# StanfordVL/RubiksNet

Hardware: AMD Instinct MI355X
Metric: RubiksShift3D fwd+bwd GB/s vs HBM roofline (higher is better)
Workload: dtype f32

## Files before the change

include/rubiks_hip.h:

```cpp
#ifndef RUBIKS_HIP_H_
#define RUBIKS_HIP_H_

#include <stddef.h>

#ifdef __cplusplus
extern "C" {
#endif

typedef void* rk_stream_t;

enum {
    RK_OK = 0,
    RK_ERR_NULL_POINTER = -1,
    RK_ERR_BAD_DIMS = -2,
    RK_ERR_BAD_STRIDE = -3,
    RK_ERR_WORKSPACE = -4,
    RK_ERR_LAUNCH = -5,
    RK_ERR_NO_DEVICE = -6,
    RK_ERR_UNSUPPORTED = -7
};

int rk_version(void);
const char* rk_error_string(int code);
int rk_out_len(int in, int stride, int pad);
// ... 238 lines not shown
                         int quantize, void* workspace, size_t workspace_bytes, rk_stream_t stream);
int rk_pw_tiles(int F, int P);
int rk_pw_gemm_tiles(const float* A, int F, int K, int M, int P, int a_is_mk);
int rk_pw2_gemm_cfg_f32(const float* A, const float* X, const float* R, float* Y, int F, int K, int M, int P, int a_is_mk,
                        const float* ka, const float* kb, int relu_in, int rb, int amode, int ct, rk_stream_t stream);
int rk_pw4_gemm_f32(const float* A, const float* X, const float* R, float* Y, int F, int K, int M, int P, int a_is_mk,
                    const float* ka, const float* kb, int relu_in, int epi, void* stats, const float* bx, const float* bpack,
                    void* bred, int tiles, rk_stream_t stream);
size_t rk_pw2_wgrad_workspace_bytes(int F, int K, int M, int P);
int rk_pw2_wgrad_cfg_f32(const float* dY, const float* X, float* dW, int F, int K, int M, int P, void* ws, size_t ws_bytes,
                         const float* ka, const float* kb, int relu_in, int inst, int stages, int splits, rk_stream_t stream);
int rk_pw_gemm_stats_f32(const float* A, const float* X, const float* R, float* Y, int F, int K, int M, int P,
                         int a_is_mk, const float* ka, const float* kb, int relu_in, void* stats, int tiles,
                         rk_stream_t stream);
int rk_stem_conv3x3s2_stats_f32(const float* W, const float* X, float* Y, int F, int Cin, int Cout, int Hin, int Win,
                                void* stats, int tiles, rk_stream_t stream);
int rk_pw_gemm_bnbwd_f32(const float* A, const float* dY, const float* R, float* dZ, int F, int K, int M, int P,
                         int a_is_mk, const float* x, const float* abmi , void* bred,
                         int tiles, rk_stream_t stream);
int rk_pw_wgrad_pro_f32(const float* dY, const float* X, float* dW, int F, int K, int M, int P, const float* ka,
                        const float* kb, int relu_in, void* ws, size_t ws_bytes, rk_stream_t stream);
int rk_pw_s2_wgrad_pro_f32(const float* dY, const float* X, float* dW, int F, int Cin, int Cout, int Hin, int Win,
                           const float* ka, const float* kb, int relu_in, void* ws, size_t ws_bytes, rk_stream_t stream);
int rk_bn_finish_tiles_f32(const void* stats, int tiles, long long count, const float* gamma, const float* beta,
                           float* running_mean, float* running_var, float* save_mean, float* save_invstd, float* a,
                           float* b, float* abmi , int C, float eps, float momentum,
                           long long* num_batches_tracked, rk_stream_t stream);
int rk_bn_tile_stats_f32(const float* x, void* stats, int F, int C, int P, rk_stream_t stream);
int rk_bn_apply_affine_bf16(const void* x, const float* a, const float* b, void* y, int F, int C, int P, int relu,
                            rk_stream_t stream);
int rk_bn_apply_affine_f32(const float* x, const float* a, const float* b, float* y, int F, int C, int P, int relu,
                           rk_stream_t stream);
int rk_bn_bwd_finish_tiles_f32(const void* bred, int tiles, long long count, float* k12, float* dgamma, float* dbeta,
                               int C, rk_stream_t stream);
int rk_bn_bwd_dx_pre_f32(const float* dz, const float* x, const float* gamma, const float* save_mean,
                         const float* save_invstd, const float* k12, const float* skip, float* dx, int F, int C, int P,
                         rk_stream_t stream);
int rk_bn_bwd_dx_pre_bf16(const void* dz, const void* x, const float* gamma, const float* save_mean,
                          const float* save_invstd, const float* k12, const void* skip, void* dx, int F, int C, int P,
                          rk_stream_t stream);
int rk_bn_stats_finish_f32(const float* x, const float* gamma, const float* beta, float* running_mean, float* running_var,
                           float* save_mean, float* save_invstd, float* ab, int F, int C, int P, float eps, float momentum,
                           long long* num_batches_tracked, void* ws, size_t ws_bytes, rk_stream_t stream);
int rk_bn_stats_finish_bf16(const void* x, const float* gamma, const float* beta, float* running_mean, float* running_var,
                            float* save_mean, float* save_invstd, float* ab, int F, int C, int P, float eps, float momentum,
                            long long* num_batches_tracked, void* ws, size_t ws_bytes, rk_stream_t stream);
// ... 34 lines not shown
```

rubiksnet_amd/_native.py:

```python
import ctypes
import os
import threading

_HERE = os.path.dirname(os.path.abspath(__file__))
LIB_PATH = os.environ.get("RK_HIP_LIB") or os.path.join(_HERE, "csrc", "librubiks_hip.so")

_lock = threading.Lock()
_lib = None

_i = ctypes.c_int
_p = ctypes.c_void_p
_sz = ctypes.c_size_t

_DIMS3 = [_i] * 5 + [_i] * 6
_DIMS2 = [_i] * 4 + [_i] * 4
SIGNATURES = {
    "rk_version": (_i, []),
    "rk_error_string": (ctypes.c_char_p, [_i]),
    "rk_out_len": (_i, [_i, _i, _i]),
    "rk_device_count": (_i, []),
    "rk_debug_peek_launch_tag": (ctypes.c_uint, []),
    "rk_debug_set_finalize_spins": (_i, [_i]),
    "rk3d_debug_finalize_only_f32": (_i, [_p, _sz, _i, _i, _p, _i, ctypes.c_float, _p]),
    "rk3d_forward_f32": (_i, [_p, _p, _p] + _DIMS3 + [_i, _p]),
# ... 58 lines not shown
    "rk_pw_wgrad_workspace_bytes": (_sz, [_i, _i, _i, _i]),
    "rk_pw2_gemm_cfg_f32": (_i, [_p, _p, _p, _p, _i, _i, _i, _i, _i, _p, _p, _i, _i, _i, _i, _p]),
    "rk_pw4_gemm_f32": (_i, [_p, _p, _p, _p, _i, _i, _i, _i, _i, _p, _p, _i, _i, _p, _p, _p, _p, _i, _p]),
    "rk_pw2_wgrad_workspace_bytes": (_sz, [_i, _i, _i, _i]),
    "rk_pw2_wgrad_cfg_f32": (_i, [_p, _p, _p, _i, _i, _i, _i, _p, _sz, _p, _p, _i, _i, _i, _i, _p]),
    "rk_pw_wgrad_f32": (_i, [_p, _p, _p, _i, _i, _i, _i, _p, _sz, _p]),
    "rk_pw_wgrad_bf16": (_i, [_p, _p, _p, _i, _i, _i, _i, _p, _sz, _p]),
    "rk_pw_gemm_odd_f32": (_i, [_p, _p, _p, _p, _i, _i, _i, _i, _i, _p]),
    "rk_pw_wgrad_odd_workspace_bytes": (_sz, [_i, _i, _i, _i]),
    "rk_pw_wgrad_odd_f32": (_i, [_p, _p, _p, _i, _i, _i, _i, _p, _sz, _p]),
    "rk_pw_s2_forward_odd_f32": (_i, [_p, _p, _p, _i, _i, _i, _i, _i, _p]),
    "rk_pw_s2_dgrad_odd_f32": (_i, [_p, _p, _p, _i, _i, _i, _i, _i, _p]),
    "rk_pw_s2_wgrad_odd_f32": (_i, [_p, _p, _p, _i, _i, _i, _i, _i, _p, _sz, _p]),
    "rk3d_forward_bn_f32": (_i, [_p, _p, _p, _p] + _DIMS3 + [_i, _p]),
    "rk3d_backward_bn_workspace_bytes": (_sz, _DIMS3),
    "rk3d_backward_bn_f32": (_i, [_p] * 9 + _DIMS3 + [_i, ctypes.c_float, _i, _p, _sz, _p]),
    "rk_pw_tiles": (_i, [_i, _i]),
    "rk_pw_gemm_tiles": (_i, [_p, _i, _i, _i, _i, _i]),
    "rk_pw_gemm_stats_f32": (_i, [_p, _p, _p, _p, _i, _i, _i, _i, _i, _p, _p, _i, _p, _i, _p]),
    "rk_stem_conv3x3s2_stats_f32": (_i, [_p, _p, _p, _i, _i, _i, _i, _i, _p, _i, _p]),
    "rk_pw_gemm_bnbwd_f32": (_i, [_p, _p, _p, _p, _i, _i, _i, _i, _i, _p, _p, _p, _i, _p]),
    "rk_pw_wgrad_pro_f32": (_i, [_p, _p, _p, _i, _i, _i, _i, _p, _p, _i, _p, _sz, _p]),
    "rk_pw_s2_wgrad_pro_f32": (_i, [_p, _p, _p, _i, _i, _i, _i, _i, _p, _p, _i, _p, _sz, _p]),
    "rk_bn_finish_tiles_f32": (_i, [_p, _i, ctypes.c_longlong, _p, _p, _p, _p, _p, _p, _p, _p, _p, _i, ctypes.c_float,
                                    ctypes.c_float, _p, _p]),
    "rk_bn_tile_stats_f32": (_i, [_p, _p, _i, _i, _i, _p]),
    "rk_bn_apply_affine_f32": (_i, [_p, _p, _p, _p, _i, _i, _i, _i, _p]),
    "rk_bn_apply_affine_bf16": (_i, [_p, _p, _p, _p, _i, _i, _i, _i, _p]),
    "rk_bn_bwd_finish_tiles_f32": (_i, [_p, _i, ctypes.c_longlong, _p, _p, _p, _i, _p]),
    "rk_bn_bwd_dx_pre_f32": (_i, [_p, _p, _p, _p, _p, _p, _p, _p, _i, _i, _i, _p]),
    "rk_bn_bwd_dx_pre_bf16": (_i, [_p, _p, _p, _p, _p, _p, _p, _p, _i, _i, _i, _p]),
    "rk_bn_stats_finish_f32": (_i, [_p, _p, _p, _p, _p, _p, _p, _p, _i, _i, _i, ctypes.c_float, ctypes.c_float, _p, _p, _sz, _p]),
    "rk_bn_stats_finish_bf16": (_i, [_p, _p, _p, _p, _p, _p, _p, _p, _i, _i, _i, ctypes.c_float, ctypes.c_float, _p, _p, _sz, _p]),
    "rk_bn_stats_finish_abmi_f32": (_i, [_p] * 9 + [_i, _i, _i, ctypes.c_float, ctypes.c_float, _p, _p, _sz, _p]),
    "rk_bn_stats_finish_abmi_bf16": (_i, [_p] * 9 + [_i, _i, _i, ctypes.c_float, ctypes.c_float, _p, _p, _sz, _p]),
}
SIGNATURES["rk_se_mlp_forward_f32"] = (_i, [_p, _p, _p, _p, _p, _i, _i, _i, _p])
SIGNATURES["rk_se_mlp_backward_f32"] = (_i, [_p] * 11 + [_i, _i, _i, _p])
SIGNATURES["rk_se_dgate_f32"] = (_i, [_p, _p, _p, _i, _i, _i, _p])
SIGNATURES["rk_se_scale_add_f32"] = (_i, [_p, _p, _p, ctypes.c_float, _p, _i, _i, _i, _p])
for _sfx in ("f32", "bf16"):
    SIGNATURES["rk_clip_u8_to_chw_" + _sfx] = (_i, [_p, _p, _p, _p, _i, _i, _i, _i, _p])
    SIGNATURES["rk_se_squeeze_" + _sfx] = (_i, [_p, _p, _i, _i, _i, _p])
    SIGNATURES["rk_se_scale_" + _sfx] = (_i, [_p, _p, _p, _i, _i, _i, _p])
    SIGNATURES["rk_se_scale_backward_" + _sfx] = (_i, [_p, _p, _p, _p, _p, _i, _i, _i, _p])
    SIGNATURES["rk_bn_relu_forward_" + _sfx] = (
# ... 53 lines not shown
```

rubiksnet_amd/csrc/rk_pw4.hip:

```cpp
#include <type_traits>
#include "rk_common.hpp"
#include "rk_dma.hpp"
#include "rk_pw4.hpp"

namespace rk {
namespace pw4 {

typedef float f32x4 __attribute__((ext_vector_type(4)));

struct Dims {
    int F, K, M, P;
    long long ntot;
    long long ntiles;
    int a_is_mk;
};

#ifndef RK_PW4_NT
#define RK_PW4_NT 2
#endif
#if RK_PW4_NT & 1
#define RK_PW4_LDNT " nt"
#else
#define RK_PW4_LDNT ""
#endif
__device__ __forceinline__ void dma16v(const void* p, unsigned lds_dst_uniform) {
    unsigned keep;
    asm volatile(
        "s_mov_b32 %0, m0\n\t"
        "s_mov_b32 m0, %2\n\t"
        "s_waitcnt lgkmcnt(0)\n\t"
        "global_load_lds_dwordx4 %1, off" RK_PW4_LDNT "\n\t"
        "s_mov_b32 m0, %0"
        : "=&s"(keep)
        : "v"(p), "s"(lds_dst_uniform)
        : "memory");
}
__device__ __forceinline__ float row16_sum_to_lane15(float v) {
// ... 25 lines not shown
    int n = 0;
    for (int u = a; u <= b; ++u) {
        int uu = u;
        if (u < 0) {
            if (first) continue;
            uu = u + NRT;
        }
        if (ne0) n += uu == NRT - 1 ? 4 * (RB - 1) * ns : 0;
        else if (uu >= NST && uu < NST + NE && (uu - NST) / 4 < RB - 1) n += ns;
    }
    return n;
}
constexpr int best_div(int n, int maxrec) {
    for (int dd = maxrec; dd >= 2; --dd)
        if (n % dd == 0) return dd;
    return 1;
}
constexpr int pad_of(int n, int maxrec) {
    for (int p = 0; p < 8; ++p)
        if (best_div(n + p, maxrec) >= 8) return p;
    return 0;
}
constexpr int maxrec_of(bool ALDS) { return ALDS ? 17 : 19; }

template <int RB, int NST, bool PRO, int EPI, bool RES, bool ALDS>
__global__ __launch_bounds__(64 * waves_of(ALDS), ALDS ? 1 : 2) void k_pw4_gemm(const float* __restrict__ A, const float* __restrict__ X,
                                                             const float* __restrict__ R, float* __restrict__ Y, Dims d,
                                                             pw2::GFuse fz, pw2::GTrain tr) {
    static_assert(!(EPI == 2 && (RES || PRO)), "no such instance");
    constexpr int NE = (EPI == 2 || RES) ? 4 * RB : 0;
    constexpr int NPAD = pad_of(NST + NE, maxrec_of(ALDS));
    constexpr int NRT = NST + NE + NPAD;
    constexpr int NREC = best_div(NRT, maxrec_of(ALDS));
    constexpr int LOOK = NREC - 1;
    constexpr int NS = EPI == 0 ? 1 : 2;
    static_assert(LOOK >= 2 && LOOK <= NRT, "ring");
    constexpr int kWaves = waves_of(ALDS);
    extern __shared__ __attribute__((aligned(16))) float lds_f[];
    const int wave = __builtin_amdgcn_readfirstlane((int)(threadIdx.x >> 6)), lane = threadIdx.x & 63;
    const int j = lane & 15, kq = lane >> 4;
    float* ring = lds_f + wave * (NREC * 256);
    float2* Ks = reinterpret_cast<float2*>(lds_f + kWaves * NREC * 256);
    float4* Bp = reinterpret_cast<float4*>(lds_f + kWaves * NREC * 256 + 8 * NST);
    float* At = lds_f + kWaves * NREC * 256 + 8 * NST + 64 * RB;
    const int K = d.K, M = d.M, P = d.P;
    if constexpr (ALDS) {
        for (int e = threadIdx.x; e < RB * NST * 64; e += 64 * kWaves) {
            const int l = e & 63, fs = e >> 6, st = fs % NST, rb = fs / NST;
            const int m = 16 * rb + (l & 15), k = 4 * st + (l >> 4);
            const bool ok = m < M && k < K;
            const size_t at = d.a_is_mk ? (size_t)m * K + k : (size_t)k * M + m;
            const float v = A[ok ? at : 0];
            At[e] = ok ? v : 0.f;
        }
    }
    if constexpr (PRO) {
        for (int e = threadIdx.x; e < 4 * NST; e += 64 * kWaves)
            Ks[e] = e < K ? make_float2(fz.ka[e], fz.kb[e]) : make_float2(0.f, 0.f);
    }
    if constexpr (EPI == 2) {
        for (int e = threadIdx.x; e < 16 * RB; e += 64 * kWaves) Bp[e] = tr.bpack[e < M ? e : M - 1];
    }
    const bool outaff = EPI == 0 && fz.ma != nullptr;
    if (outaff) {
        for (int e = threadIdx.x; e < 16 * RB; e += 64 * kWaves) {
            const int m = e < M ? e : M - 1;
            Bp[e] = make_float4(fz.ma[m], fz.mb[m], 0.f, 0.f);
        }
    }
    if (PRO || EPI == 2 || ALDS || outaff) __syncthreads();

    const int gw = blockIdx.x * kWaves + wave, nwv = gridDim.x * kWaves;
    if (gw >= d.ntiles) return;
    const int ntw = (int)((d.ntiles - gw + nwv - 1) / nwv);

    const float* E = EPI == 2 ? tr.bx : R;
    const unsigned cstep = 64u * (unsigned)nwv, df = cstep / (unsigned)P, dp = cstep - df * (unsigned)P;
    unsigned pf_, pp_;
    {
        unsigned c = (unsigned)gw * 64u + 4u * (unsigned)j;
        c = c < (unsigned)d.ntot ? c : 0u;
        pf_ = c / (unsigned)P; pp_ = c - pf_ * (unsigned)P;
    }
    int ptile = 0;
    const unsigned ring_b = dma::lds_byte_addr(ring);
    const size_t kqP = (size_t)kq * P;
    int xfix;
    {
        const int k = 4 * (NST - 1) + kq;
        xfix = ((k < K ? k : K - 1) - k) * P;
    }
    const float* xp = nullptr;
    const float* ep = nullptr;
    size_t yo_next = 0;
    auto enter_tile = [&]() {
        const unsigned f = (pf_ * (unsigned)P + pp_) < (unsigned)d.ntot ? pf_ : 0u, p = f == pf_ ? pp_ : 0u;
        xp = X + ((size_t)f * K) * P + p + kqP;
        yo_next = ((size_t)f * M) * P + p;
        if constexpr (NE > 0) ep = E + yo_next + 4 * kqP;
// ... 37 lines not shown
    static_for<LOOK>([&](auto I) { issue(I); });
    size_t yo_c = yo_next, yo_next_c = yo_next;

    float a[ALDS ? 1 : RB][ALDS ? 1 : NST];
    if constexpr (!ALDS) {
#pragma unroll
        for (int rb = 0; rb < RB; ++rb)
#pragma unroll
            for (int st = 0; st < NST; ++st) {
                const int m = 16 * rb + j, k = 4 * st + kq;
                const bool ok = m < M && k < K;
                const size_t at = d.a_is_mk ? (size_t)m * K + k : (size_t)k * M + m;
                const float v = A[ok ? at : 0];
                a[rb][st] = ok ? v : 0.f;
            }
    }
    float acur[RB];
    auto read_a = [&](auto STc, float (&dst)[RB]) {
        constexpr int st = decltype(STc)::value;
#pragma unroll
        for (int rb = 0; rb < RB; ++rb) dst[rb] = At[(rb * NST + st) * 64 + lane];
    };
    if constexpr (ALDS) read_a(std::integral_constant<int, 0>{}, acur);

    asm volatile("s_waitcnt vmcnt(%0)" ::"n"(LOOK - 1) : "memory");
    f32x4 vcur = read_rec(std::integral_constant<int, 0>{});

    int t = 0;
    auto tile_body = [&](auto FIRSTc) {
        constexpr bool FIRST = decltype(FIRSTc)::value;
        const long long tg = (long long)gw + (long long)t * nwv;
        const bool valid = tg * 64 + 4 * j < d.ntot;
        const long long nleft = d.ntot - tg * 64;
        const float ntile = (float)(nleft < 64 ? nleft : 64);
        float* yp = Y + yo_c + 4 * kqP;
        size_t rec = (size_t)(4 * kq) * tr.J + (size_t)tg;
        auto finish_row = [&](auto RBc, auto Rc, const f32x4& ev) {
            constexpr int rb = decltype(RBc)::value, r = decltype(Rc)::value;
            const int m = 16 * rb + 4 * kq + r;
            const bool live = rb < RB - 1 || m < M;
            const bool on = valid && live;
            float4 o = make_float4(acc[rb][0][r], acc[rb][1][r], acc[rb][2][r], acc[rb][3][r]);
            if constexpr (EPI == 0) {
                if (outaff) {
                    const float4 pk = Bp[16 * rb + 4 * kq + r];
                    o.x = fmaf(pk.x, o.x, pk.y); o.y = fmaf(pk.x, o.y, pk.y); o.z = fmaf(pk.x, o.z, pk.y); o.w = fmaf(pk.x, o.w, pk.y);
// ... 18 lines not shown
                    const float4 pk = Bp[16 * rb + 4 * kq + r];
                    if (on) {
                        const float pa = pk.x, pb = pk.y, mu = pk.z, iv = pk.w;
                        o.x = fmaf(pa, ev[0], pb) <= 0.f ? 0.f : o.x;  s1 += o.x;  s2 = fmaf(o.x, (ev[0] - mu) * iv, s2);
                        o.y = fmaf(pa, ev[1], pb) <= 0.f ? 0.f : o.y;  s1 += o.y;  s2 = fmaf(o.y, (ev[1] - mu) * iv, s2);
                        o.z = fmaf(pa, ev[2], pb) <= 0.f ? 0.f : o.z;  s1 += o.z;  s2 = fmaf(o.z, (ev[2] - mu) * iv, s2);
                        o.w = fmaf(pa, ev[3], pb) <= 0.f ? 0.f : o.w;  s1 += o.w;  s2 = fmaf(o.w, (ev[3] - mu) * iv, s2);
                    }
                }
                if (on) store_y(yp, o);
                s1 = row16_sum_to_lane15(s1);
                s2 = row16_sum_to_lane15(s2);
                if (j == 15 && live) {
                    if constexpr (EPI == 1) tr.stats[rec] = make_float4(piv, s1, s2, ntile);
                    else tr.bred[rec] = make_float2(s1, s2);
                }
                rec += (r == 3 ? 13 : 1) * (size_t)tr.J;
            }
            yp += (r == 3 ? 13 : 1) * (size_t)P;
        };

        static_for<NRT>([&](auto S) {
            constexpr int s = decltype(S)::value;
            issue(std::integral_constant<int, (s + LOOK) % NRT>{});
            if constexpr ((s + LOOK) % NRT == 0) yo_next_c = yo_next;
            constexpr int W = (LOOK - 1) + certain_stores(s + 1 - LOOK, s - 1, FIRST, NRT, NST, NE, RB, NS);
            static_assert(W <= 63, "vmcnt is 6 bits");
            asm volatile("s_waitcnt vmcnt(%0)" ::"n"(W) : "memory");
            const f32x4 vnext = read_rec(std::integral_constant<int, (s + 1) % NRT>{});
            const f32x4 v = vcur;
            float anext[RB];
            if constexpr (ALDS && ((s + 1) % NRT) < NST) read_a(std::integral_constant<int, (s + 1) % NRT>{}, anext);
            if constexpr (s < NST) {
                float b[4] = {v[0], v[1], v[2], v[3]};
                if constexpr (PRO) {
                    const float2 kk = Ks[4 * s + kq];
#pragma unroll
                    for (int q = 0; q < 4; ++q) {
                        const float tq = fmaf(kk.x, b[q], kk.y);
                        b[q] = fz.relu_in ? fmaxf(tq, 0.f) : tq;
                    }
                }
#pragma unroll
                for (int rb = 0; rb < RB; ++rb)
#pragma unroll
                    for (int q = 0; q < 4; ++q)
// ... 2 lines not shown
                constexpr int e = s - NST;
                finish_row(std::integral_constant<int, e / 4>{}, std::integral_constant<int, e % 4>{}, v);
            }
            vcur = vnext;
            if constexpr (ALDS && ((s + 1) % NRT) < NST) {
#pragma unroll
                for (int rb = 0; rb < RB; ++rb) acur[rb] = anext[rb];
            }
        });
        if constexpr (NE == 0) {
            static_for<4 * RB>([&](auto Ec) {
                constexpr int e = decltype(Ec)::value;
                finish_row(std::integral_constant<int, e / 4>{}, std::integral_constant<int, e % 4>{}, f32x4{0.f, 0.f, 0.f, 0.f});
            });
        }
#pragma unroll
        for (int rb = 0; rb < RB; ++rb)
#pragma unroll
            for (int q = 0; q < 4; ++q) acc[rb][q] = f32x4{0.f, 0.f, 0.f, 0.f};
        yo_c = yo_next_c;
    };
    tile_body(std::true_type{});
    for (t = 1; t < ntw; ++t) tile_body(std::false_type{});
}

struct Inst { int rb, nst; };
inline bool pick(Inst& in, int K, int M) {
    const int nrb = (M + 15) / 16, nst = (K + 3) / 4;
    if (nrb == 4 && nst >= 12 && nst <= 14) { in = Inst{4, 14}; return true; }
    if (nrb == 5 && nst >= 16 && nst <= 18) { in = Inst{5, 18}; return true; }
    return false;
}
inline int mode() {
    static const int m = [] { const char* e = getenv("RK_PW4"); return e ? atoi(e) : 1; }();
    return m;
}
inline int num_cus() { return device_cus(); }
constexpr long long kMinTiles = 4096;

template <int RB, int NST, bool PRO, int EPI, bool RES>
int launch(const float* A, const float* X, const float* R, float* Y, const Dims& d, const pw2::GFuse& fz, const pw2::GTrain& tr,
           hipStream_t stream) {
    constexpr bool ALDS = RB == 5 && EPI != 0;
    constexpr int NE = (EPI == 2 || RES) ? 4 * RB : 0;
    constexpr int NREC = best_div(NST + NE + pad_of(NST + NE, maxrec_of(ALDS)), maxrec_of(ALDS));
    constexpr int kWaves = waves_of(ALDS);
    if ((long long)d.F * d.K * d.P < 256) return RK_ERR_UNSUPPORTED;
    constexpr int wgs_per_cu = ALDS ? 1 : 2;
    const size_t lds = (size_t)kWaves * NREC * 1024 + 8 * NST * sizeof(float) + 16 * RB * sizeof(float4) +
                       (ALDS ? (size_t)RB * NST * 256 : 0);
    if (lds > 160 * 1024) return RK_ERR_UNSUPPORTED;
    static DynLdsRaised raised;
    if (const int rc = raise_dynamic_lds(reinterpret_cast<const void*>(&k_pw4_gemm<RB, NST, PRO, EPI, RES, ALDS>), lds, raised))
        return rc;
    long long wgs = (long long)num_cus() * wgs_per_cu;
    const long long need = (d.ntiles + kWaves - 1) / kWaves;
    wgs = wgs < need ? wgs : need;
    hipLaunchKernelGGL((k_pw4_gemm<RB, NST, PRO, EPI, RES, ALDS>), dim3((unsigned)wgs), dim3(64 * kWaves), lds, stream, A, X, R, Y, d,
                       fz, tr);
    return launch_status();
}
template <int RB, int NST>
int launch_flags(int pro, int epi, int res, const float* A, const float* X, const float* R, float* Y, const Dims& d,
                 const pw2::GFuse& fz, const pw2::GTrain& tr, hipStream_t stream) {
    if (epi == 2) {
        if (pro || res) return RK_ERR_UNSUPPORTED;
        return launch<RB, NST, false, 2, false>(A, X, R, Y, d, fz, tr, stream);
    }
#define RK_P4(E) do { \
        if (pro) return res ? launch<RB, NST, true, E, true>(A, X, R, Y, d, fz, tr, stream) \
                            : launch<RB, NST, true, E, false>(A, X, R, Y, d, fz, tr, stream); \
        return res ? launch<RB, NST, false, E, true>(A, X, R, Y, d, fz, tr, stream) \
                   : launch<RB, NST, false, E, false>(A, X, R, Y, d, fz, tr, stream); } while (0)
    if (epi == 1) RK_P4(1);
    RK_P4(0);
#undef RK_P4
}

long long tiles(int F, int K, int M, int P, int epi, int res, bool force) {
    if (F <= 0 || K <= 0 || M <= 0 || P <= 0 || P % 4 != 0 || (long long)F * P >= (1ll << 31)) return 0;
    if (mode() == 0) return 0;
    Inst in;
    if (!pick(in, K, M)) return 0;
    const long long nt = ((long long)F * P + 63) / 64;
    if (!force && mode() != 2) {
        if (nt < kMinTiles) return 0;
        if (in.rb == 5 && epi == 1 && res) return 0;
    }
    return nt;
}

int gemm(const float* A, const float* X, const float* R, float* Y, int F, int K, int M, int P, int a_is_mk, const pw2::GFuse* fuse,
         const pw2::GTrain* train, int epi, hipStream_t stream, bool force) {
    if (!A || !X || !Y) return RK_ERR_NULL_POINTER;
    if (F <= 0 || K <= 0 || M <= 0 || P <= 0 || P % 4 != 0) return RK_ERR_BAD_DIMS;
    if (((uintptr_t)X & 15) || ((uintptr_t)Y & 15) || (R && ((uintptr_t)R & 15))) return RK_ERR_BAD_DIMS;
    Inst in;
    if (!pick(in, K, M)) return RK_ERR_UNSUPPORTED;
    if (tiles(F, K, M, P, epi, R != nullptr, force) <= 0) return RK_ERR_UNSUPPORTED;
    pw2::GFuse fz = fuse ? *fuse : pw2::GFuse{nullptr, nullptr, nullptr, nullptr, 0, 0};
    pw2::GTrain tr = train ? *train : pw2::GTrain{nullptr, nullptr, nullptr, nullptr, 0};
    if (fz.ma && (epi != 0 || !fz.mb)) return RK_ERR_UNSUPPORTED;
    const int pro = fz.ka != nullptr, res = R != nullptr;
    Dims d;
    d.F = F; d.K = K; d.M = M; d.P = P; d.ntot = (long long)F * P; d.ntiles = (d.ntot + 63) / 64; d.a_is_mk = a_is_mk;
    if (epi == 1 && !tr.stats) return RK_ERR_NULL_POINTER;
    if (epi == 2 && !(tr.bred && tr.bx && tr.bpack)) return RK_ERR_NULL_POINTER;
    if (epi == 2 && ((uintptr_t)tr.bx & 15)) return RK_ERR_BAD_DIMS;
    if (epi && (long long)tr.J != d.ntiles) return RK_ERR_BAD_DIMS;
    if (in.rb == 4) return launch_flags<4, 14>(pro, epi, res, A, X, R, Y, d, fz, tr, stream);
    return launch_flags<5, 18>(pro, epi, res, A, X, R, Y, d, fz, tr, stream);
}

}
}

extern "C" {
using namespace rk;
int rk_pw4_gemm_f32(const float* A, const float* X, const float* R, float* Y, int F, int K, int M, int P, int a_is_mk,
                    const float* ka, const float* kb, int relu_in, int epi, void* stats, const float* bx, const float* bpack,
                    void* bred, int tiles, rk_stream_t stream) {
    const pw2::GFuse fz{ka, kb, nullptr, nullptr, relu_in, 0};
    const pw2::GTrain tr{(float4*)stats, (float2*)bred, bx, (const float4*)bpack, tiles};
    return pw4::gemm(A, X, R, Y, F, K, M, P, a_is_mk, &fz, &tr, epi, (hipStream_t)stream, true);
}
}
```

rubiksnet_amd/train_block.py:

```python
import logging

import torch

from . import _native, config, rubiksnet_cuda
from .fused_bn import _count_batch

__all__ = ["fused_train_block", "take_stats", "bn_relu_from_stats", "stats_fallbacks"]

_LOG = logging.getLogger("rubiksnet_amd")
_FALLBACKS = [0]


def stats_fallbacks():
    return _FALLBACKS[0]


def _note_fallback(shape):
    _FALLBACKS[0] += 1
    if _FALLBACKS[0] == 1:
        _LOG.warning("rubiksnet_amd: a fused training block received x %s without its producer's BatchNorm tile statistics "
                     "and runs a statistics pass of its own (logged once; train_block.stats_fallbacks() counts them)",
                     tuple(shape))

_CMAX = 320
# ... 210 lines not shown
        s3, pd = [1, plan.stride, plan.stride], [0, 0, 0]
        if dout is None:
            return (None,) * 13
        dout = dout.contiguous()
        need = ctx.needs_input_grad
        with torch.cuda.device(dev):
            st = _stream(dev)
            cur = torch.cuda.current_stream(dev)
            side = _side_stream(dev)
            keep = []

            def wgrad_ws(K, M, Pn):
                nbytes = int(L.rk_pw_wgrad_workspace_bytes(Fr, K, M, Pn))
                buf = torch.empty(max(nbytes, 1), dtype=torch.uint8, device=dev)
                keep.append(buf)
                return buf, nbytes

            def wg_stream():
                if side is None:
                    return st
                side.wait_stream(cur)
                return side.cuda_stream

            try:
                ds = torch.empty_like(s)
                _native.check(L.rk_pw_gemm_f32(w3.data_ptr(), dout.data_ptr(), None, ds.data_ptr(), Fr, Cout, Cmid, Po, 0, st),
                              "rk_pw_gemm_f32")
                dw3 = None
                if need[8]:
                    dw3 = torch.empty_like(w3)
                    ws, nb = wgrad_ws(Cmid, Cout, Po)
                    _native.check(L.rk_pw_wgrad_f32(dout.data_ptr(), (s_in if ctx.has_se else s).data_ptr(), dw3.data_ptr(), Fr,
                                                    Cmid, Cout, Po, ws.data_ptr(), nb, wg_stream()), "rk_pw_wgrad_f32")
                if ctx.has_se:
                    dgate = torch.empty_like(se_g)
                    _native.check(L.rk_se_dgate_f32(ds.data_ptr(), s.data_ptr(), dgate.data_ptr(), Fr, Cmid, Po, st),
                                  "rk_se_dgate_f32")
                    Cr = wse1.shape[0]
                    dpre2 = torch.empty_like(se_g)
                    dpre1 = torch.empty_like(se_h)
                    dq = torch.empty_like(se_g)
                    dwse1, dwse2 = torch.empty_like(wse1), torch.empty_like(wse2)
                    rc = L.rk_se_mlp_backward_f32(dgate.data_ptr(), se_g.data_ptr(), se_h.data_ptr(), se_q.data_ptr(), wse1.data_ptr(),
                                                  wse2.data_ptr(), dpre2.data_ptr(), dpre1.data_ptr(), dq.data_ptr(), dwse1.data_ptr(),
                                                  dwse2.data_ptr(), Fr, Cmid, Cr, st)
                    if rc == rubiksnet_cuda.UNSUPPORTED:
                        dpre2 = dgate * se_g * (1.0 - se_g)
                        dwse2 = dpre2.t() @ se_h
                        dpre1 = (dpre2 @ wse2) * (se_h > 0).to(dpre2.dtype)
                        dwse1 = dpre1.t() @ se_q
                        dq = (dpre1 @ wse1).contiguous()
                    else:
# ... 39 lines not shown
                if not need[7]:
                    dshift = None
                res, dwsc = None, None
                if not plan.identity:
                    res = torch.empty_like(x)
                    if plan.stride == 2:
                        _native.check(L.rk_pw_s2_dgrad_f32(wsc.data_ptr(), dout.data_ptr(), res.data_ptr(), Fr, Cin, Cout, H, W,
                                                           st), "rk_pw_s2_dgrad_f32")
                    else:
                        _native.check(L.rk_pw_gemm_f32(wsc.data_ptr(), dout.data_ptr(), None, res.data_ptr(), Fr, Cout, Cin, P,
                                                       0, st), "rk_pw_gemm_f32")
                    if need[9]:
                        dwsc = torch.empty_like(wsc)
                        ws, nb = wgrad_ws(Cin, Cout, Po)
                        if plan.stride == 2:
                            _native.check(L.rk_pw_s2_wgrad_pro_f32(dout.data_ptr(), x.data_ptr(), dwsc.data_ptr(), Fr, Cin, Cout,
                                                                   H, W, bn1[2].data_ptr(), bn1[3].data_ptr(), 1, ws.data_ptr(),
                                                                   nb, wg_stream()), "rk_pw_s2_wgrad_pro_f32")
                        else:
                            _native.check(L.rk_pw_wgrad_pro_f32(dout.data_ptr(), x.data_ptr(), dwsc.data_ptr(), Fr, Cin, Cout, P,
                                                                bn1[2].data_ptr(), bn1[3].data_ptr(), 1, ws.data_ptr(), nb,
                                                                wg_stream()), "rk_pw_wgrad_pro_f32")
                dw2 = None
                if need[4]:
                    dw2 = torch.empty_like(w2)
                    ws, nb = wgrad_ws(Cin, Cmid, P)
                    _native.check(L.rk_pw_wgrad_pro_f32(dz.data_ptr(), x.data_ptr(), dw2.data_ptr(), Fr, Cin, Cmid, P,
                                                        bn1[2].data_ptr(), bn1[3].data_ptr(), 1, ws.data_ptr(), nb, wg_stream()),
                                  "rk_pw_wgrad_pro_f32")
                J = int(L.rk_pw_gemm_tiles(w2.data_ptr(), Fr, Cmid, Cin, P, 0))
                bred = torch.empty(Cin, J, 2, dtype=torch.float32, device=dev)
                dzm = res if res is not None else torch.empty_like(x)
                _native.check(L.rk_pw_gemm_bnbwd_f32(w2.data_ptr(), dz.data_ptr(), _ptr(res), dzm.data_ptr(), Fr, Cmid, Cin, P,
                                                     0, x.data_ptr(), bn1[4].data_ptr(), bred.data_ptr(), J, st),
                              "rk_pw_gemm_bnbwd_f32")
                k12 = torch.empty(2, Cin, dtype=torch.float32, device=dev)
                dg1 = torch.empty(Cin, dtype=torch.float32, device=dev)
                db1 = torch.empty(Cin, dtype=torch.float32, device=dev)
                _native.check(L.rk_bn_bwd_finish_tiles_f32(bred.data_ptr(), J, Fr * P, k12.data_ptr(), dg1.data_ptr(),
                                                           db1.data_ptr(), Cin, st), "rk_bn_bwd_finish_tiles_f32")
                dx = None
                if need[0]:
                    dx = torch.empty_like(x)
                    skip = dout if plan.identity else None
                    _native.check(L.rk_bn_bwd_dx_pre_f32(dzm.data_ptr(), x.data_ptr(), g1.data_ptr(), bn1[0].data_ptr(),
                                                         bn1[1].data_ptr(), k12.data_ptr(), _ptr(skip), dx.data_ptr(), Fr, Cin,
                                                         P, st), "rk_bn_bwd_dx_pre_f32")
            finally:
                if side is not None:
                    cur.wait_stream(side)
                del keep
        return (dx, None, dg1, db1, dw2, dg2, db2, dshift, dw3, dwsc if not plan.identity else None, dwse1, dwse2, None)


def fused_train_block(block, x):
    sw = config.switches()
    if not (sw.fused_train and sw.fused_bn and sw.pointwise != "0"):
        return None
# ... 91 lines not shown
```

Before: 5821.

## Fuse pointwise dgrad GEMM with weight-gradient accumulation in backward pass

Adds a WG variant of the pw4 GEMM kernel. While streaming dY tiles to compute dX, it also reads the matching activation (E) tiles from the ring buffer and accumulates the weight gradient with MFMA into per-wave partials, which a reduce kernel then sums. The training block uses this fused path for the w3 and w2 (BN-backward with prologue affine) backward GEMMs by default, falling back when unsupported. This removes the separate wgrad kernel's re-read of dY and X from HBM. In exchange, occupancy drops to one workgroup per CU, register pressure rises, the partial workspace is extra traffic, and the wgrad no longer runs overlapped on a side stream.

After: 5816 (median of 6 runs). Within noise of the previous version (-0.1%).

```diff
diff --git a/include/rubiks_hip.h b/include/rubiks_hip.h
--- a/include/rubiks_hip.h
+++ b/include/rubiks_hip.h
@@ -284,6 +284,17 @@
                         const float* kb, int relu_in, void* ws, size_t ws_bytes, rk_stream_t stream);
 int rk_pw_s2_wgrad_pro_f32(const float* dY, const float* X, float* dW, int F, int Cin, int Cout, int Hin, int Win,
                            const float* ka, const float* kb, int relu_in, void* ws, size_t ws_bytes, rk_stream_t stream);
+size_t rk_pw_gemm_wgrad_workspace_bytes(int F, int K, int M, int P);
+int rk_pw_gemm_wgrad_f32(const float* A, const float* dY, float* dZ, int F, int K, int M, int P, int a_is_mk, const float* X,
+                         float* dW, void* ws, size_t ws_bytes, rk_stream_t stream);
+size_t rk_pw_gemm_bnbwd_wgrad_pro_workspace_bytes(int F, int K, int M, int P);
+int rk_pw_gemm_bnbwd_wgrad_pro_f32(const float* A, const float* dY, float* dZ, int F, int K, int M, int P, int a_is_mk,
+                                   const float* x, const float* abmi, void* bred, int tiles, const float* ka, const float* kb,
+                                   int relu_in, float* dW, void* ws, size_t ws_bytes, rk_stream_t stream);
+size_t rk_pw4_gemm_wgrad_workspace_bytes(int F, int K, int M, int P);
+int rk_pw4_gemm_wgrad_f32(const float* A, const float* dY, float* dZ, int F, int K, int M, int P, int a_is_mk, const float* bx,
+                          const float* abmi, void* bred, int tiles, const float* E, const float* ka, const float* kb, int relu_in,
+                          float* dW, void* ws, size_t ws_bytes, rk_stream_t stream);
 int rk_bn_finish_tiles_f32(const void* stats, int tiles, long long count, const float* gamma, const float* beta,
                            float* running_mean, float* running_var, float* save_mean, float* save_invstd, float* a,
                            float* b, float* abmi , int C, float eps, float momentum,
diff --git a/rubiksnet_amd/_native.py b/rubiksnet_amd/_native.py
--- a/rubiksnet_amd/_native.py
+++ b/rubiksnet_amd/_native.py
@@ -104,6 +104,12 @@
     "rk_pw_gemm_bnbwd_f32": (_i, [_p, _p, _p, _p, _i, _i, _i, _i, _i, _p, _p, _p, _i, _p]),
     "rk_pw_wgrad_pro_f32": (_i, [_p, _p, _p, _i, _i, _i, _i, _p, _p, _i, _p, _sz, _p]),
     "rk_pw_s2_wgrad_pro_f32": (_i, [_p, _p, _p, _i, _i, _i, _i, _i, _p, _p, _i, _p, _sz, _p]),
+    "rk_pw_gemm_wgrad_workspace_bytes": (_sz, [_i, _i, _i, _i]),
+    "rk_pw_gemm_wgrad_f32": (_i, [_p, _p, _p, _i, _i, _i, _i, _i, _p, _p, _p, _sz, _p]),
+    "rk_pw_gemm_bnbwd_wgrad_pro_workspace_bytes": (_sz, [_i, _i, _i, _i]),
+    "rk_pw_gemm_bnbwd_wgrad_pro_f32": (_i, [_p, _p, _p, _i, _i, _i, _i, _i, _p, _p, _p, _i, _p, _p, _i, _p, _p, _sz, _p]),
+    "rk_pw4_gemm_wgrad_workspace_bytes": (_sz, [_i, _i, _i, _i]),
+    "rk_pw4_gemm_wgrad_f32": (_i, [_p, _p, _p, _i, _i, _i, _i, _i, _p, _p, _p, _i, _p, _p, _p, _i, _p, _p, _sz, _p]),
     "rk_bn_finish_tiles_f32": (_i, [_p, _i, ctypes.c_longlong, _p, _p, _p, _p, _p, _p, _p, _p, _p, _i, ctypes.c_float,
                                     ctypes.c_float, _p, _p]),
     "rk_bn_tile_stats_f32": (_i, [_p, _p, _i, _i, _i, _p]),
diff --git a/rubiksnet_amd/csrc/rk_pw4.hip b/rubiksnet_amd/csrc/rk_pw4.hip
--- a/rubiksnet_amd/csrc/rk_pw4.hip
+++ b/rubiksnet_amd/csrc/rk_pw4.hip
@@ -2,6 +2,7 @@
 #include "rk_common.hpp"
 #include "rk_dma.hpp"
 #include "rk_pw4.hpp"
+#include "rk_reduce.hpp"
 
 namespace rk {
 namespace pw4 {
@@ -13,6 +14,12 @@
     long long ntot;
     long long ntiles;
     int a_is_mk;
+};
+struct WgArgs {
+    const float* E;
+    const float* ka; const float* kb;
+    int relu_in;
+    float* part;
 };
 
 #ifndef RK_PW4_NT
@@ -84,17 +91,21 @@
     return 0;
 }
 constexpr int maxrec_of(bool ALDS) { return ALDS ? 17 : 19; }
-
-template <int RB, int NST, bool PRO, int EPI, bool RES, bool ALDS>
-__global__ __launch_bounds__(64 * waves_of(ALDS), ALDS ? 1 : 2) void k_pw4_gemm(const float* __restrict__ A, const float* __restrict__ X,
+constexpr int maxrec_of(bool ALDS, int WG) { return WG ? 32 : maxrec_of(ALDS); }
+
+template <int RB, int NST, bool PRO, int EPI, bool RES, bool ALDS, int WG = 0>
+__global__ __launch_bounds__(64 * waves_of(ALDS), (ALDS || WG) ? 1 : 2) void k_pw4_gemm(const float* __restrict__ A, const float* __restrict__ X,
                                                              const float* __restrict__ R, float* __restrict__ Y, Dims d,
-                                                             pw2::GFuse fz, pw2::GTrain tr) {
+                                                             pw2::GFuse fz, pw2::GTrain tr, WgArgs wg) {
     static_assert(!(EPI == 2 && (RES || PRO)), "no such instance");
-    constexpr int NE = (EPI == 2 || RES) ? 4 * RB : 0;
-    constexpr int NPAD = pad_of(NST + NE, maxrec_of(ALDS));
+    static_assert(!(WG && (PRO || RES || ALDS || EPI == 1)), "no such instance");
+    constexpr int NE = (EPI == 2 || RES || WG) ? 4 * RB : 0;
+    constexpr int NPAD = pad_of(NST + NE, maxrec_of(ALDS, WG));
     constexpr int NRT = NST + NE + NPAD;
-    constexpr int NREC = best_div(NRT, maxrec_of(ALDS));
-    constexpr int LOOK = NREC - 1;
+    constexpr int NREC = best_div(NRT, maxrec_of(ALDS, WG));
+    constexpr int LOOK = WG ? NREC - 3 : NREC - 1;
+    constexpr int KB = (NST + 3) / 4;
+    static_assert(!WG || NPAD == 0, "WG: no padding records");
     constexpr int NS = EPI == 0 ? 1 : 2;
     static_assert(LOOK >= 2 && LOOK <= NRT, "ring");
     constexpr int kWaves = waves_of(ALDS);
@@ -105,6 +116,7 @@
     float2* Ks = reinterpret_cast<float2*>(lds_f + kWaves * NREC * 256);
     float4* Bp = reinterpret_cast<float4*>(lds_f + kWaves * NREC * 256 + 8 * NST);
     float* At = lds_f + kWaves * NREC * 256 + 8 * NST + 64 * RB;
+    float2* Kw = reinterpret_cast<float2*>(lds_f + kWaves * NREC * 256 + 8 * NST + 64 * RB);
     const int K = d.K, M = d.M, P = d.P;
     if constexpr (ALDS) {
         for (int e = threadIdx.x; e < RB * NST * 64; e += 64 * kWaves) {
@@ -130,13 +142,23 @@
             Bp[e] = make_float4(fz.ma[m], fz.mb[m], 0.f, 0.f);
         }
     }
-    if (PRO || EPI == 2 || ALDS || outaff) __syncthreads();
+    if constexpr (WG == 2) {
+        for (int e = threadIdx.x; e < 16 * RB; e += 64 * kWaves)
+            Kw[e] = e < M ? make_float2(wg.ka[e], wg.kb[e]) : make_float2(0.f, 0.f);
+    }
+    if (PRO || EPI == 2 || ALDS || outaff || WG == 2) __syncthreads();
 
     const int gw = blockIdx.x * kWaves + wave, nwv = gridDim.x * kWaves;
-    if (gw >= d.ntiles) return;
+    if (gw >= d.ntiles) {
+        if constexpr (WG != 0) {
+            float* pp = wg.part + (size_t)gw * K * M;
+            for (int e = lane; e < K * M; e += 64) pp[e] = 0.f;
+        }
+        return;
+    }
     const int ntw = (int)((d.ntiles - gw + nwv - 1) / nwv);
 
-    const float* E = EPI == 2 ? tr.bx : R;
+    const float* E = EPI == 2 ? tr.bx : (WG ? wg.E : R);
     const unsigned cstep = 64u * (unsigned)nwv, df = cstep / (unsigned)P, dp = cstep - df * (unsigned)P;
     unsigned pf_, pp_;
     {
@@ -220,6 +242,25 @@
         for (int rb = 0; rb < RB; ++rb) dst[rb] = At[(rb * NST + st) * 64 + lane];
     };
     if constexpr (ALDS) read_a(std::integral_constant<int, 0>{}, acur);
+
+    auto read_t = [&](auto R0c, auto NRc, auto EPc, f32x4 (&dst)[4]) {
+        constexpr int R0 = decltype(R0c)::value, NR = decltype(NRc)::value;
+        constexpr bool EP = decltype(EPc)::value;
+        int rr = EP ? (j & 3) : (j >> 2);
+        const int rin = EP ? (j >> 2) : (j & 3);
+        if constexpr (NR < 4) rr = rr < NR ? rr : NR - 1;
+        int sl = R0 % NREC + rr;
+        if constexpr (R0 % NREC + 3 >= NREC) sl = sl >= NREC ? sl - NREC : sl;
+        const float* base = ring + sl * 256 + (rin * 16 + kq) * 4;
+#pragma unroll
+        for (int c = 0; c < 4; ++c) dst[c] = *reinterpret_cast<const f32x4*>(base + 16 * c);
+    };
+    f32x4 dyT[WG ? KB : 1][4];
+    f32x4 dwacc[WG ? KB : 1][WG ? RB : 1];
+#pragma unroll
+    for (int kb = 0; kb < (WG ? KB : 1); ++kb)
+#pragma unroll
+        for (int mb = 0; mb < (WG ? RB : 1); ++mb) dwacc[kb][mb] = f32x4{0.f, 0.f, 0.f, 0.f};
 
     asm volatile("s_waitcnt vmcnt(%0)" ::"n"(LOOK - 1) : "memory");
     f32x4 vcur = read_rec(std::integral_constant<int, 0>{});
@@ -284,6 +325,36 @@
 
         static_for<NRT>([&](auto S) {
             constexpr int s = decltype(S)::value;
+            if constexpr (WG != 0 && s < NST && (s % 4 == 3 || s == NST - 1)) {
+                read_t(std::integral_constant<int, s / 4 * 4>{}, std::integral_constant<int, s - s / 4 * 4 + 1>{},
+                       std::false_type{}, dyT[s / 4]);
+            } else if constexpr (WG != 0 && s >= NST && s < NST + NE && (s - NST) % 4 == 3) {
+                constexpr int mb = (s - NST) / 4;
+                f32x4 eT[4];
+                read_t(std::integral_constant<int, s - 3>{}, std::integral_constant<int, 4>{}, std::true_type{}, eT);
+                float2 kk = make_float2(1.f, 0.f);
+                if constexpr (WG == 2) kk = Kw[16 * mb + j];
+#pragma unroll
+                for (int c = 0; c < 4; ++c) {
+                    const bool ok = 16 * c + 4 * kq < nleft;
+#pragma unroll
+                    for (int q = 0; q < 4; ++q) {
+                        float e = eT[c][q];
+                        if constexpr (WG == 2) {
+                            e = fmaf(kk.x, e, kk.y);
+                            e = wg.relu_in ? fmaxf(e, 0.f) : e;
+                        }
+                        eT[c][q] = ok ? e : 0.f;
+                    }
+                }
+#pragma unroll
+                for (int c = 0; c < 4; ++c)
+#pragma unroll
+                    for (int q = 0; q < 4; ++q)
+#pragma unroll
+                        for (int kb = 0; kb < KB; ++kb)
+                            dwacc[kb][mb] = __builtin_amdgcn_mfma_f32_16x16x4f32(dyT[kb][c][q], eT[c][q], dwacc[kb][mb], 0, 0, 0);
+            }
             issue(std::integral_constant<int, (s + LOOK) % NRT>{});
             if constexpr ((s + LOOK) % NRT == 0) yo_next_c = yo_next;
             constexpr int W = (LOOK - 1) + certain_stores(s + 1 - LOOK, s - 1, FIRST, NRT, NST, NE, RB, NS);
@@ -332,6 +403,18 @@
     };
     tile_body(std::true_type{});
     for (t = 1; t < ntw; ++t) tile_body(std::false_type{});
+    if constexpr (WG != 0) {
+        float* pp = wg.part + (size_t)gw * K * M;
+#pragma unroll
+        for (int kb = 0; kb < KB; ++kb)
+#pragma unroll
+            for (int mb = 0; mb < RB; ++mb)
+#pragma unroll
+                for (int r = 0; r < 4; ++r) {
+                    const int k = 16 * kb + 4 * kq + r, m = 16 * mb + j;
+                    if (k < K && m < M) pp[(size_t)k * M + m] = dwacc[kb][mb][r];
+                }
+    }
 }
 
 struct Inst { int rb, nst; };
@@ -348,26 +431,32 @@
 inline int num_cus() { return device_cus(); }
 constexpr long long kMinTiles = 4096;
 
-template <int RB, int NST, bool PRO, int EPI, bool RES>
+template <bool ALDS, int WG>
+long long grid_of(const Dims& d) {
+    constexpr int kWaves = waves_of(ALDS);
+    constexpr int wgs_per_cu = (ALDS || WG) ? 1 : 2;
+    long long wgs = (long long)num_cus() * wgs_per_cu;
+    const long long need = (d.ntiles + kWaves - 1) / kWaves;
+    return wgs < need ? wgs : need;
+}
+
+template <int RB, int NST, bool PRO, int EPI, bool RES, int WG = 0>
 int launch(const float* A, const float* X, const float* R, float* Y, const Dims& d, const pw2::GFuse& fz, const pw2::GTrain& tr,
-           hipStream_t stream) {
-    constexpr bool ALDS = RB == 5 && EPI != 0;
-    constexpr int NE = (EPI == 2 || RES) ? 4 * RB : 0;
-    constexpr int NREC = best_div(NST + NE + pad_of(NST + NE, maxrec_of(ALDS)), maxrec_of(ALDS));
+           hipStream_t stream, const WgArgs& wg = WgArgs{nullptr, nullptr, nullptr, 0, nullptr}) {
+    constexpr bool ALDS = RB == 5 && EPI != 0 && WG == 0;
+    constexpr int NE = (EPI == 2 || RES || WG) ? 4 * RB : 0;
+    constexpr int NREC = best_div(NST + NE + pad_of(NST + NE, maxrec_of(ALDS, WG)), maxrec_of(ALDS, WG));
     constexpr int kWaves = waves_of(ALDS);
     if ((long long)d.F * d.K * d.P < 256) return RK_ERR_UNSUPPORTED;
-    constexpr int wgs_per_cu = ALDS ? 1 : 2;
     const size_t lds = (size_t)kWaves * NREC * 1024 + 8 * NST * sizeof(float) + 16 * RB * sizeof(float4) +
-                       (ALDS ? (size_t)RB * NST * 256 : 0);
+                       (ALDS ? (size_t)RB * NST * 256 : 0) + (WG ? 16 * RB * sizeof(float2) : 0);
     if (lds > 160 * 1024) return RK_ERR_UNSUPPORTED;
     static DynLdsRaised raised;
-    if (const int rc = raise_dynamic_lds(reinterpret_cast<const void*>(&k_pw4_gemm<RB, NST, PRO, EPI, RES, ALDS>), lds, raised))
+    if (const int rc = raise_dynamic_lds(reinterpret_cast<const void*>(&k_pw4_gemm<RB, NST, PRO, EPI, RES, ALDS, WG>), lds, raised))
         return rc;
-    long long wgs = (long long)num_cus() * wgs_per_cu;
-    const long long need = (d.ntiles + kWaves - 1) / kWaves;
-    wgs = wgs < need ? wgs : need;
-    hipLaunchKernelGGL((k_pw4_gemm<RB, NST, PRO, EPI, RES, ALDS>), dim3((unsigned)wgs), dim3(64 * kWaves), lds, stream, A, X, R, Y, d,
-                       fz, tr);
+    const long long wgs = grid_of<ALDS, WG>(d);
+    hipLaunchKernelGGL((k_pw4_gemm<RB, NST, PRO, EPI, RES, ALDS, WG>), dim3((unsigned)wgs), dim3(64 * kWaves), lds, stream, A, X, R, Y,
+                       d, fz, tr, wg);
     return launch_status();
 }
 template <int RB, int NST>
@@ -398,6 +487,58 @@
         if (in.rb == 5 && epi == 1 && res) return 0;
     }
     return nt;
+}
+
+inline bool fused_on() {
+    static const int m = [] { const char* e = getenv("RK_PW_FUSED_BWD"); return e ? atoi(e) : 1; }();
+    return m != 0;
+}
+long long fused_partials(int F, int K, int M, int P, bool force) {
+    if (!force && !fused_on()) return 0;
+    Inst in;
+    if (!pick(in, K, M) || (K * M) % 4 != 0) return 0;
+    if (tiles(F, K, M, P, 0, 0, force) <= 0 || (long long)F * K * P < 256) return 0;
+    Dims d;
+    d.ntot = (long long)F * P; d.ntiles = (d.ntot + 63) / 64;
+    return grid_of<false, 1>(d) * waves_of(false);
+}
+size_t fused_workspace_bytes(int F, int K, int M, int P, bool force) {
+    return (size_t)fused_partials(F, K, M, P, force) * K * M * sizeof(float);
+}
+
+int gemm_wgrad(const float* A, const float* X, float* Y, int F, int K, int M, int P, int a_is_mk, const pw2::GTrain* train, int epi,
+               const float* E, const float* ka, const float* kb, int relu_in, float* dW, void* ws, size_t ws_bytes,
+               hipStream_t stream, bool force) {
+    if (!A || !X || !Y || !dW || !E) return RK_ERR_NULL_POINTER;
+    if (F <= 0 || K <= 0 || M <= 0 || P <= 0 || P % 4 != 0) return RK_ERR_BAD_DIMS;
+    if (((uintptr_t)X & 15) || ((uintptr_t)Y & 15) || ((uintptr_t)E & 15)) return RK_ERR_BAD_DIMS;
+    if ((ka == nullptr) != (kb == nullptr)) return RK_ERR_NULL_POINTER;
+    const bool pro = ka != nullptr;
+    if (!(epi == 0 && !pro) && !(epi == 2 && pro)) return RK_ERR_UNSUPPORTED;
+    Inst in;
+    if (!pick(in, K, M) || (K * M) % 4 != 0) return RK_ERR_UNSUPPORTED;
+    const long long S = fused_partials(F, K, M, P, force);
+    if (S <= 0) return RK_ERR_UNSUPPORTED;
+    const size_t need = (size_t)S * K * M * sizeof(float);
+    if (!ws || ws_bytes < need || ((uintptr_t)ws & 15) || ((uintptr_t)dW & 15)) return RK_ERR_WORKSPACE;
+    pw2::GTrain tr = train ? *train : pw2::GTrain{nullptr, nullptr, nullptr, nullptr, 0};
+    const pw2::GFuse fz{nullptr, nullptr, nullptr, nullptr, 0, 0};
+    Dims d;
+    d.F = F; d.K = K; d.M = M; d.P = P; d.ntot = (long long)F * P; d.ntiles = (d.ntot + 63) / 64; d.a_is_mk = a_is_mk;
+    if (epi == 2) {
+        if (!(tr.bred && tr.bx && tr.bpack)) return RK_ERR_NULL_POINTER;
+        if (tr.bx != E) return RK_ERR_BAD_DIMS;
+        if ((long long)tr.J != d.ntiles) return RK_ERR_BAD_DIMS;
+    }
+    const WgArgs wg{E, ka, kb, relu_in, (float*)ws};
+    int rc;
+    if (in.rb == 4) rc = epi == 2 ? launch<4, 14, false, 2, false, 2>(A, X, nullptr, Y, d, fz, tr, stream, wg)
+                                  : launch<4, 14, false, 0, false, 1>(A, X, nullptr, Y, d, fz, tr, stream, wg);
+    else rc = epi == 2 ? launch<5, 18, false, 2, false, 2>(A, X, nullptr, Y, d, fz, tr, stream, wg)
+                       : launch<5, 18, false, 0, false, 1>(A, X, nullptr, Y, d, fz, tr, stream, wg);
+    if (rc) return rc;
+    launch_reduce_partials4((const float*)ws, dW, K * M, (int)S, stream);
+    return launch_status();
 }
 
 int gemm(const float* A, const float* X, const float* R, float* Y, int F, int K, int M, int P, int a_is_mk, const pw2::GFuse* fuse,
@@ -434,4 +575,28 @@
     const pw2::GTrain tr{(float4*)stats, (float2*)bred, bx, (const float4*)bpack, tiles};
     return pw4::gemm(A, X, R, Y, F, K, M, P, a_is_mk, &fz, &tr, epi, (hipStream_t)stream, true);
 }
-}
+size_t rk_pw4_gemm_wgrad_workspace_bytes(int F, int K, int M, int P) { return pw4::fused_workspace_bytes(F, K, M, P, true); }
+int rk_pw4_gemm_wgrad_f32(const float* A, const float* dY, float* dZ, int F, int K, int M, int P, int a_is_mk, const float* bx,
+                          const float* abmi, void* bred, int tiles, const float* E, const float* ka, const float* kb, int relu_in,
+                          float* dW, void* ws, size_t ws_bytes, rk_stream_t stream) {
+    const pw2::GTrain tr{nullptr, (float2*)bred, bx, (const float4*)abmi, tiles};
+    return pw4::gemm_wgrad(A, dY, dZ, F, K, M, P, a_is_mk, &tr, bx ? 2 : 0, E, ka, kb, relu_in, dW, ws, ws_bytes, (hipStream_t)stream,
+                           true);
+}
+
+size_t rk_pw_gemm_wgrad_workspace_bytes(int F, int K, int M, int P) { return pw4::fused_workspace_bytes(F, K, M, P, false); }
+size_t rk_pw_gemm_bnbwd_wgrad_pro_workspace_bytes(int F, int K, int M, int P) {
+    return pw4::fused_workspace_bytes(F, K, M, P, false);
+}
+int rk_pw_gemm_wgrad_f32(const float* A, const float* dY, float* dZ, int F, int K, int M, int P, int a_is_mk, const float* X,
+                         float* dW, void* ws, size_t ws_bytes, rk_stream_t stream) {
+    return pw4::gemm_wgrad(A, dY, dZ, F, K, M, P, a_is_mk, nullptr, 0, X, nullptr, nullptr, 0, dW, ws, ws_bytes,
+                           (hipStream_t)stream, false);
+}
+int rk_pw_gemm_bnbwd_wgrad_pro_f32(const float* A, const float* dY, float* dZ, int F, int K, int M, int P, int a_is_mk,
+                                   const float* x, const float* abmi, void* bred, int tiles, const float* ka, const float* kb,
+                                   int relu_in, float* dW, void* ws, size_t ws_bytes, rk_stream_t stream) {
+    const pw2::GTrain tr{nullptr, (float2*)bred, x, (const float4*)abmi, tiles};
+    return pw4::gemm_wgrad(A, dY, dZ, F, K, M, P, a_is_mk, &tr, 2, x, ka, kb, relu_in, dW, ws, ws_bytes, (hipStream_t)stream, false);
+}
+}
diff --git a/rubiksnet_amd/train_block.py b/rubiksnet_amd/train_block.py
--- a/rubiksnet_amd/train_block.py
+++ b/rubiksnet_amd/train_block.py
@@ -256,12 +256,29 @@
                 side.wait_stream(cur)
                 return side.cuda_stream
 
+            def fused_ws(query, K, M, Pn):
+                nbytes = int(query(Fr, K, M, Pn))
+                if nbytes <= 0:
+                    return None, 0
+                return torch.empty(nbytes, dtype=torch.uint8, device=dev), nbytes
+
             try:
                 ds = torch.empty_like(s)
-                _native.check(L.rk_pw_gemm_f32(w3.data_ptr(), dout.data_ptr(), None, ds.data_ptr(), Fr, Cout, Cmid, Po, 0, st),
-                              "rk_pw_gemm_f32")
                 dw3 = None
+                fused3 = False
                 if need[8]:
+                    wsf, nb = fused_ws(L.rk_pw_gemm_wgrad_workspace_bytes, Cout, Cmid, Po)
+                    if wsf is not None:
+                        dw3 = torch.empty_like(w3)
+                        rc = L.rk_pw_gemm_wgrad_f32(w3.data_ptr(), dout.data_ptr(), ds.data_ptr(), Fr, Cout, Cmid, Po, 0,
+                                                    (s_in if ctx.has_se else s).data_ptr(), dw3.data_ptr(), wsf.data_ptr(), nb, st)
+                        fused3 = rc != rubiksnet_cuda.UNSUPPORTED
+                        if fused3:
+                            _native.check(rc, "rk_pw_gemm_wgrad_f32")
+                if not fused3:
+                    _native.check(L.rk_pw_gemm_f32(w3.data_ptr(), dout.data_ptr(), None, ds.data_ptr(), Fr, Cout, Cmid, Po, 0,
+                                                   st), "rk_pw_gemm_f32")
+                if need[8] and not fused3:
                     dw3 = torch.empty_like(w3)
                     ws, nb = wgrad_ws(Cmid, Cout, Po)
                     _native.check(L.rk_pw_wgrad_f32(dout.data_ptr(), (s_in if ctx.has_se else s).data_ptr(), dw3.data_ptr(), Fr,
@@ -347,18 +364,31 @@
                                                                 bn1[2].data_ptr(), bn1[3].data_ptr(), 1, ws.data_ptr(), nb,
                                                                 wg_stream()), "rk_pw_wgrad_pro_f32")
                 dw2 = None
-                if need[4]:
-                    dw2 = torch.empty_like(w2)
-                    ws, nb = wgrad_ws(Cin, Cmid, P)
-                    _native.check(L.rk_pw_wgrad_pro_f32(dz.data_ptr(), x.data_ptr(), dw2.data_ptr(), Fr, Cin, Cmid, P,
-                                                        bn1[2].data_ptr(), bn1[3].data_ptr(), 1, ws.data_ptr(), nb, wg_stream()),
-                                  "rk_pw_wgrad_pro_f32")
                 J = int(L.rk_pw_gemm_tiles(w2.data_ptr(), Fr, Cmid, Cin, P, 0))
                 bred = torch.empty(Cin, J, 2, dtype=torch.float32, device=dev)
                 dzm = res if res is not None else torch.empty_like(x)
-                _native.check(L.rk_pw_gemm_bnbwd_f32(w2.data_ptr(), dz.data_ptr(), _ptr(res), dzm.data_ptr(), Fr, Cmid, Cin, P,
-                                                     0, x.data_ptr(), bn1[4].data_ptr(), bred.data_ptr(), J, st),
-                              "rk_pw_gemm_bnbwd_f32")
+                fused2 = False
+                if need[4] and res is None:
+                    wsf, nb = fused_ws(L.rk_pw_gemm_bnbwd_wgrad_pro_workspace_bytes, Cmid, Cin, P)
+                    if wsf is not None:
+                        dw2 = torch.empty_like(w2)
+                        rc = L.rk_pw_gemm_bnbwd_wgrad_pro_f32(w2.data_ptr(), dz.data_ptr(), dzm.data_ptr(), Fr, Cmid, Cin, P, 0,
+                                                              x.data_ptr(), bn1[4].data_ptr(), bred.data_ptr(), J,
+                                                              bn1[2].data_ptr(), bn1[3].data_ptr(), 1, dw2.data_ptr(),
+                                                              wsf.data_ptr(), nb, st)
+                        fused2 = rc != rubiksnet_cuda.UNSUPPORTED
+                        if fused2:
+                            _native.check(rc, "rk_pw_gemm_bnbwd_wgrad_pro_f32")
+                if not fused2:
+                    if need[4]:
+                        dw2 = torch.empty_like(w2)
+                        ws, nb = wgrad_ws(Cin, Cmid, P)
+                        _native.check(L.rk_pw_wgrad_pro_f32(dz.data_ptr(), x.data_ptr(), dw2.data_ptr(), Fr, Cin, Cmid, P,
+                                                            bn1[2].data_ptr(), bn1[3].data_ptr(), 1, ws.data_ptr(), nb,
+                                                            wg_stream()), "rk_pw_wgrad_pro_f32")
+                    _native.check(L.rk_pw_gemm_bnbwd_f32(w2.data_ptr(), dz.data_ptr(), _ptr(res), dzm.data_ptr(), Fr, Cmid, Cin,
+                                                         P, 0, x.data_ptr(), bn1[4].data_ptr(), bred.data_ptr(), J, st),
+                                  "rk_pw_gemm_bnbwd_f32")
                 k12 = torch.empty(2, Cin, dtype=torch.float32, device=dev)
                 dg1 = torch.empty(Cin, dtype=torch.float32, device=dev)
                 db1 = torch.empty(Cin, dtype=torch.float32, device=dev)
```
